# hdm0922/PathTracerDemo

Hardware: AMD Instinct MI355X
Metric: Msamples/sec at 1920x1080, 1 spp ReSTIR DI; per-pixel L2 vs WebGPU ref (higher is better)
Workload: dtype f32; 1 GPU; c3_interior_32 reuse 1920x1080, 1 spp/frame (configs[2]); frame=1920x1080, band_rows_per_gpu=1080, parallelism=row-bands x1

## Files before the change

### pathtracerdemo_amd/csrc/ptx_launch.h

```cpp
#pragma once

#include <hip/hip_runtime.h>

#include "ptx_device.h"

namespace ptx {

constexpr int kTile = 16;
constexpr int kBlock = 256;

int env_knob(const char *key, int dflt);
#ifdef PTX_AB_BUILD
inline int ab_knob(const char *key, int dflt) { return env_knob(key, dflt); }
#else
constexpr int ab_knob(const char *, int dflt) { return dflt; }
#endif

inline size_t stack_lds_bytes(uint32_t depth) { return (size_t)depth * kBlock * sizeof(uint32_t); }

hipError_t launch_gbuffer(const Scene &sc, uint4 *gbuf, uint32_t stack_depth, hipStream_t s);
hipError_t launch_init(const Scene &sc, const uint4 *gbuf, uint4 *reservoir, uint32_t stack_depth, hipStream_t s);
hipError_t launch_final(const Scene &sc, const uint4 *gbuf, const uint4 *reservoir, float4 *accum,
                        uint32_t stack_depth, hipStream_t s);
hipError_t launch_mcpt(const Scene &sc, float4 *accum, uint32_t stack_depth, hipStream_t s);
hipError_t launch_present(const float4 *tex, uint32_t W, uint32_t H, uint32_t cw, uint32_t ch, bool bgra,
                          uint32_t *out, hipStream_t s);

hipError_t launch_trace_rays(const Scene &sc, const float4 *rays, float4 *hits, uint32_t n, int eps_mode,
                             uint32_t stack_depth, hipStream_t s);

constexpr uint32_t kWaveStateSlots = 10u;
constexpr uint32_t kStateCs2 = 7u, kStateCs3 = 8u, kStateTsel = 9u;
constexpr uint32_t kWaveSegPixels = 768u;
constexpr int kWaveRoundsInit = 3, kWaveRoundsFinal = 3, kWaveRoundsMcpt = 4;
constexpr int kWaveMaxRounds = 5;
constexpr uint32_t kDynHeads = 8u, kDynStride = 32u;
constexpr uint32_t kDynRoundWords = kDynHeads * kDynStride;
constexpr uint32_t kDynCounters = 2u * 4u * kWaveMaxRounds * kDynRoundWords;
struct WaveBufs {
    float4 *state;
    uint32_t npix;
    uint32_t seg_px;
    uint32_t nseg;
    uint32_t seg_base;
    uint32_t seg_count;
    uint32_t cluster;
    uint32_t ray_stride;
    float4 *rays;
    float4 *res[3];
    uint32_t nres;
    uint32_t *act[2];
    uint32_t act_stride;
    uint32_t *cnt;
    uint32_t trace_waves;
    uint32_t trace_split;
// ... 75 lines not shown
```

### pathtracerdemo_amd/csrc/ptx_reuse.hip

```cpp
#include "ptx_wave_common.h"

namespace ptx {

constexpr uint32_t SALT_TEMPORAL = 0x54454D50u, SALT_SPATIAL = 0x53504154u;

enum : uint32_t { JS_HDR, JS_F, JS_CUR, JS_NRM, JS_PREV, JS_RRF, JS_COUNT };
constexpr uint32_t kJobFresh = 1u << 24;
constexpr uint32_t kResReuseLayout = 0x100u;
#ifndef PTX_JOB_FRESH
#define PTX_JOB_FRESH 1
#endif

struct Job {
    uint32_t i, length, phase, seed1, idx, matref;
    uint32_t k, lab;
    bool shift, rok;
    int32_t ref;
    int32_t dom;
    f3 f;
    float prod;
    Surface cur;
    f3 prev;
    float beta, rr_p;
    f3 rr_f;
// ... 62 lines not shown
    } else if (s.phase != 1u) {
        const float4 cu = st[JS_CUR * n + jid], nr = st[JS_NRM * n + jid];
        const float4 pv = st[JS_PREV * n + jid], rf = st[JS_RRF * n + jid];
        matref = asu(cu.w);
        cur.pos = mk(cu.x, cu.y, cu.z);
        cur.nrm = mk(nr.x, nr.y, nr.z);
        cur.mat = material_at(sc, matref);
        beta = nr.w;
        prev = mk(pv.x, pv.y, pv.z); rr_p = pv.w;
        rr_f = mk(rf.x, rf.y, rf.z);
    }
    s.seed1 = seed1; s.matref = matref; s.dom = dom;
    s.f = f; s.rr_f = rr_f; s.prev = prev;
    s.beta = beta; s.rr_p = rr_p;
    s.cur = cur;
}

__device__ __forceinline__ bool rr_step(Job &s, const Surface &X, f3 L, f3 fv, float pdf) {
    s.rr_f = s.rr_f * (fv * fabsf(dot(X.nrm, L)));
    s.rr_p *= pdf;
    const float ps = luminance(s.rr_f) / s.rr_p;
    const bool ok = ps > 0.0f;
    s.rr_p *= ps;
    if (ps > 1.0f) s.beta /= ps;
    return ok;
}

__device__ __forceinline__ void job_init(Job &s, f3 x0, const Surface &X1, uint32_t matref, int32_t ref,
                                         uint32_t length, uint32_t seed1, int32_t dom, uint32_t k, bool shift) {
    s.i = 1u; s.length = length; s.phase = 0u; s.seed1 = seed1; s.idx = 0u; s.ref = ref; s.dom = dom;
    s.k = min(k, 7u); s.lab = 0u; s.shift = shift; s.rok = false;
    s.f = mk(1.0f, 1.0f, 1.0f); s.prod = 1.0f;
    s.prev = x0;
    s.cur = X1;
    s.matref = matref;
    s.beta = 1.0f; s.rr_p = 1.0f; s.rr_f = mk(1.0f, 1.0f, 1.0f);
}
__device__ __forceinline__ bool job_begin(const Scene &sc, const ReuseArgs &A, Job &s, uint32_t x, uint32_t y,
                                          int32_t dom, int32_t ref) {
    const uint4 *rv = res_at(A.cur, ref);
    const uint4 r5 = rv[5];
    const uint32_t C = rv[7].y, length = r5.w;
    Surface X1;
    uint32_t matref;
    if (C == 0u || length < 2u || !surf_load(sc, A.surf, dom, X1, matref)) return false;
    job_init(s, x0_of(sc, x, y), X1, matref, ref, length, rv[0].y, dom, r5.x & 0xffu, false);
    return true;
// ... 217 lines not shown
__device__ __forceinline__ void write_reused(uint4 *out, const uint4 *src, float p_sel, float q_sel, SelF fs,
                                             float w_sum, uint32_t C) {
    uint4 a0 = src[0], a5 = src[5];
    const uint4 a1 = src[1], a2 = src[2], a3 = src[3], a4 = src[4];
    if (fs.known && !(a5.x & kResReuseLayout)) {
        const uint32_t k = a5.x & 0xffu;
        if (k >= 2u && k + 1u < a5.w) a0 = src[6];
        a5.x |= kResReuseLayout;
    }
    out[0] = a0; out[1] = a1; out[2] = a2; out[3] = a3; out[4] = a4; out[5] = a5;
    out[6] = make_uint4(asu(p_sel), asu(q_sel), fs.known ? asu(fs.f.x) : 0u, fs.known ? asu(fs.f.y) : 0u);
    out[7] = make_uint4(asu(p_sel > 0.0f ? w_sum / p_sel : 0.0f), C, fs.known ? asu(fs.f.z) : 0u, fs.known ? 1u : 0u);
}

constexpr uint32_t kNbrEscape = 0xFFFFFFFFu;
__device__ __forceinline__ uint4 nbr_pack(bool valid, uint4 r5, uint4 r6, uint4 r7) {
    uint32_t w = 0u;
    const uint32_t k = r5.x & 0xffu;
    if (valid)
        w = (r5.w > 0xfu || k > 0xfu || r7.y > 0x7ffffeu) ? kNbrEscape : (1u << 31) | (r5.w << 27) | (k << 23) | r7.y;
    return make_uint4(r6.x, r6.y, r7.x, w);
}

__device__ __forceinline__ bool temporal_from_init(const Scene &sc, const WaveBufs &w, const ReuseArgs &A, Job &s,
                                                   uint32_t pix, uint32_t jid) {
    const uint4 *rv = res_at(A.cur, s.ref);
    const bool hyb = job_hyb(s);
    while (s.i + 1u < s.length) {
        f3 V = normalize(s.prev - s.cur.pos);
        uint32_t seed = s.i == 1u ? rv[0].x : s.seed1, lobe;
        const f3 dir = sample_bsdf(seed, s.cur, V, lobe);
        float pdf;
        const f3 fv = bsdf_pdf(s.cur, V, dir, pdf);
        if (!hyb || s.i + 2u <= s.k) s.prod *= pdf;
        if (!rr_step(s, s.cur, dir, fv, pdf)) {
            A.jres[jid] = make_float4(0.0f, 0.0f, 0.0f, 0.0f);
            return false;
        }
        const float4 c = w.state[(s.i == 1u ? kStateCs2 : kStateCs3) * w.npix + pix];
        const Surface next = get_surface(sc, gdecode(make_uint4(asu(c.x), asu(c.y), asu(c.z), asu(c.w))));
        V = normalize(s.prev - s.cur.pos);
        const f3 L = normalize(next.pos - s.cur.pos);
        s.f = s.f * (bsdf(s.cur, L, V) * fabsf(dot(s.cur.nrm, L)));
        if (hyb && s.i + 1u == s.k) s.prod = s.prod * rc_geo(s.cur.pos, next);
        s.prev = s.cur.pos;
        s.cur = next;
        s.i += 1u;
    }
    const float T = w.state[kStateTsel * w.npix + pix].x;
    if (T < 0.0f) return true;
    const LightSample XL = load_xl(rv);
    const f3 V = normalize(s.prev - s.cur.pos);
    const f3 L = direction_to_light(s.cur, XL);
    s.f = s.f * (bsdf(s.cur, L, V) * fabsf(dot(s.cur.nrm, L)));
    float gl = 1.0f;
    if (XL.type == LIGHT_RECT) {
        const f3 r = XL.pos - s.cur.pos;
        const f3 Ld = normalize(r);
        gl = fabsf(dot(get_light(sc, (uint32_t)XL.id).dir, Ld)) / dot(r, r);
    }
    s.prod = hyb ? s.prod / s.beta : s.prod / (gl * s.beta);
    const f3 Le = l_emit<true>(XL, s.cur);
    s.f = s.f * (Le * T);
    const float qv = s.prod;
    const bool valid = qv > 0.0f && qv <= 3.402823466e38f;
    A.jres[jid] = valid ? make_float4(s.f.x, s.f.y, s.f.z, qv) : make_float4(0.0f, 0.0f, 0.0f, 0.0f);
    return false;
}

__global__ __launch_bounds__(WB) __attribute__((amdgpu_waves_per_eu(2, 8)))
void wtemporal_start(Scene sc, WaveBufs w, ReuseArgs A) {
    PTX_WAVE_TIMER(sc, KID_TEMP_START | (w.seg_base ? 0x80u : 0u));
    __shared__ uint32_t lds[3];
    const JobLists JL = job_lists(w, lds);
    const Seg g = seg_begin(w, 0u, lds);
    const uint32_t np = padded_pixels(sc);
    for (uint32_t k = 0; k < w.seg_px; k += WB) {
        const uint32_t q = seg_pixel(w, g.j, k);
        uint32_t x, y, pix = 0u;
        bool active = false;
        Job s;
        if (q < np && tile_xy(sc, q, x, y)) {
            pix = (y - sc.row_begin) * sc.width + x;
            active = job_begin(sc, A, s, x, y, (int32_t)pix, (int32_t)pix);
            if (active && A.use_init) active = temporal_from_init(sc, w, A, s, pix, pix);
        }
        const bool live = job_emit(sc, g, A, active, s, pix, active ? A.cur[8u * (size_t)pix].x : 0u);
        job_finish(g, JL, A, live, s, pix);
    }
    job_seg_end(w, g, JL);
}

__global__ __launch_bounds__(WB) void wtemporal_combine(Scene sc, WaveBufs w, ReuseArgs A) {
    PTX_WAVE_TIMER(sc, KID_TEMP_COMBINE | (w.seg_base ? 0x80u : 0u));
    const uint32_t j = w.seg_base + blockIdx.x, np = padded_pixels(sc);
    for (uint32_t k = 0; k < w.seg_px; k += WB) {
        const uint32_t q = seg_pixel(w, j, k);
        uint32_t x, y;
        if (q >= np || !tile_xy(sc, q, x, y)) continue;
        const uint32_t pix = (y - sc.row_begin) * sc.width + x;
        if (!gdecode(A.gbuf[pix]).valid) {
            A.nbr_out[pix] = make_uint4(0u, 0u, 0u, 0u);
            continue;
        }
        uint4 *rv = A.cur + 8u * (size_t)pix;
        const uint4 *hv = A.hist + 8u * (size_t)pix;
        uint32_t seed = reuse_seed(sc, x, y, SALT_TEMPORAL);
        const uint4 r5 = rv[5], r7 = rv[7];
        const float4 er = (r7.y != 0u && r5.w >= 2u) ? job_result(A, w, A.jres[pix], pix) : make_float4(0.0f, 0.0f, 0.0f, 0.0f);
        const float2 ec = make_float2(er.w > 0.0f ? luminance(mk(er.x, er.y, er.z)) : 0.0f, er.w);
        const bool canon_ok = ec.y > 0.0f && ec.x > 0.0f;
// ... 38 lines not shown
    m.py = (uint32_t)fy;
    const int32_t ry = (int32_t)m.py - (int32_t)sc.row_begin;
    if (abs((int32_t)m.py - (int32_t)y) > (int32_t)A.radius || ry < A.prev_row_lo || ry >= A.prev_row_hi) {
        if (count && A.clip) atomicAdd(A.clip, 1ull);
        return m;
    }
    m.pp = ry * (int32_t)sc.width + (int32_t)m.px;
    const uint4 a = A.psurf[2 * (ptrdiff_t)m.pp];
    if (a.w == kNoSurface) return m;
    const uint4 b = A.psurf[2 * (ptrdiff_t)m.pp + 1];
    const f3 pp = mk(asf(a.x), asf(a.y), asf(a.z)), pn = mk(asf(b.x), asf(b.y), asf(b.z));
    if (!(dot(pn, X1.nrm) >= 0.9f)) return m;
    const f3 x0p = x0_prev(A, sc, m.px, m.py);
    const float dp = length(pp - x0p), dc = length(P - x0p);
    if (!(fabsf(dp - dc) <= 0.05f * dc)) return m;
    m.C = min(A.hist[8 * (ptrdiff_t)m.pp + 7].y, A.cap);
    m.ok = m.C != 0u;
    return m;
}

#ifndef MOTION_START_WAVES
#define MOTION_START_WAVES 3
#endif
__global__ __launch_bounds__(WB) __attribute__((amdgpu_waves_per_eu(MOTION_START_WAVES, 8)))
void wtmotion_start(Scene sc, WaveBufs w, ReuseArgs A) {
    PTX_WAVE_TIMER(sc, KID_TEMP_START | (w.seg_base ? 0x80u : 0u));
    __shared__ uint32_t lds[3];
    const JobLists JL = job_lists(w, lds);
    const Seg g = seg_begin(w, 0u, lds);
    const uint32_t np = padded_pixels(sc);
    for (uint32_t k = 0; k < w.seg_px; k += WB) {
        const uint32_t q = seg_pixel(w, g.j, k);
        uint32_t x = 0u, y = 0u, pix = 0u;
        bool valid = false;
        Surface X1{};
        uint32_t mref = 0u;
        if (q < np && tile_xy(sc, q, x, y)) {
            pix = (y - sc.row_begin) * sc.width + x;
            valid = surf_load(sc, A.surf, pix, X1, mref);
        }
        const uint4 *rv = A.cur + 8u * (size_t)pix;
        const uint4 r5c = valid ? rv[5] : make_uint4(0u, 0u, 0u, 0u);
        const uint32_t cC = valid ? rv[7].y : 0u, clen = r5c.w, ck = r5c.x & 0xffu;
        const bool canon = valid && cC != 0u && clen >= 2u;
        const MotionHist mh = valid ? motion_hist(sc, A, X1, y, true) : MotionHist{false, 0, 0u, 0u, 0u};
#pragma unroll 1
        for (uint32_t slot = 0; slot < kMotionJobs; ++slot) {
            const uint32_t jid = job_id(A, pix, slot);
            Job s;
            bool act = false;
            uint32_t s0 = 0u;
            if (slot == 0u) {
                act = canon && job_begin(sc, A, s, x, y, (int32_t)pix, (int32_t)pix);
                if (act && A.use_init) act = temporal_from_init(sc, w, A, s, pix, jid);
                if (act) s0 = rv[0].x;
            } else if (slot == 1u) {
                if (mh.ok) {
                    const uint4 *hv = A.hist + 8 * (ptrdiff_t)mh.pp;
                    const uint4 h0 = hv[0], h5 = hv[5], h6 = hv[6];
                    act = h5.w >= 2u && asf(h6.x) > 0.0f;
                    if (act) {
                        job_init(s, x0_of(sc, x, y), X1, mref, kHistRef + mh.pp, h5.w, h0.y, (int32_t)pix, h5.x & 0xffu,
                                 true);
                        s0 = h0.x;
                    }
                }
            } else if (mh.ok && canon) {
                Surface Xp;
                uint32_t pref;
                act = surf_load(sc, A.psurf, mh.pp, Xp, pref);
                if (act) {
                    job_init(s, x0_prev(A, sc, mh.px, mh.py), Xp, pref, (int32_t)pix, clen, rv[0].y, kDomPrev, ck, true);
                    s0 = rv[0].x;
                }
            }
            const bool live = job_emit(sc, g, A, act, s, jid, s0);
            job_finish(g, JL, A, live, s, jid);
        }
    }
    job_seg_end(w, g, JL);
}

__global__ __launch_bounds__(WB) void wtmotion_combine(Scene sc, WaveBufs w, ReuseArgs A) {
    PTX_WAVE_TIMER(sc, KID_TEMP_COMBINE | (w.seg_base ? 0x80u : 0u));
    const uint32_t j = w.seg_base + blockIdx.x, np = padded_pixels(sc);
    for (uint32_t k = 0; k < w.seg_px; k += WB) {
        const uint32_t q = seg_pixel(w, j, k);
        uint32_t x, y;
        if (q >= np || !tile_xy(sc, q, x, y)) continue;
        const uint32_t pix = (y - sc.row_begin) * sc.width + x;
        Surface X1;
        uint32_t mref;
        if (!surf_load(sc, A.surf, pix, X1, mref)) {
            A.nbr_out[pix] = make_uint4(0u, 0u, 0u, 0u);
            continue;
        }
        uint4 *rv = A.cur + 8u * (size_t)pix;
        uint32_t seed = reuse_seed(sc, x, y, SALT_TEMPORAL);
        const uint4 r5 = rv[5], r7 = rv[7];
        const float4 er = (r7.y != 0u && r5.w >= 2u) ? job_at(A, w, pix, 0u) : make_float4(0.0f, 0.0f, 0.0f, 0.0f);
        const float ecp = er.w > 0.0f ? luminance(mk(er.x, er.y, er.z)) : 0.0f, ecq = er.w;
        const bool canon_ok = ecq > 0.0f && ecp > 0.0f;
        const float cc = 1.0f, pc = ecp, qc = ecq, Wc = asf(r7.x);
        const MotionHist mh = motion_hist(sc, A, X1, y);
// ... 90 lines not shown
    return hipGetLastError();
}

__global__ __launch_bounds__(WB) void wsurface(Scene sc, WaveBufs w, const uint4 *gbuf) {
    const uint32_t j = w.seg_base + blockIdx.x, np = padded_pixels(sc);
    for (uint32_t k = 0; k < w.seg_px; k += WB) {
        const uint32_t q = seg_pixel(w, j, k);
        uint32_t x, y;
        if (q >= np || !tile_xy(sc, q, x, y)) continue;
        const uint32_t pix = (y - sc.row_begin) * sc.width + x;
        surf_from_gbuf(sc, w.surf, (ptrdiff_t)pix, gbuf[pix]);
    }
}
hipError_t wave_surface(const Scene &sc, const WaveBufs &w, const uint4 *gbuf, hipStream_t s) {
    if (!w.surf || !w.seg_count) return hipSuccess;
    hipLaunchKernelGGL(wsurface, dim3(w.seg_count), dim3(WB), 0, s, sc, w, gbuf);
    return hipGetLastError();
}

constexpr uint32_t kMaxPrefetch = 3u;
#ifndef SPATIAL_START_WAVES
#define SPATIAL_START_WAVES 3
#endif
constexpr uint32_t kBinCap = 128u;
__device__ __forceinline__ uint32_t bin_push(uint4 *bin, uint32_t cnt, bool p, uint4 d) {
    const unsigned long long m = __ballot(p);
    const uint32_t rank = __builtin_amdgcn_mbcnt_hi((uint32_t)(m >> 32), __builtin_amdgcn_mbcnt_lo((uint32_t)m, 0u));
    if (p) bin[cnt + rank] = d;
    return cnt + (uint32_t)__popcll(m);
}
template <int KIND>
__device__ __forceinline__ void spatial_drain(const Scene &sc, const Seg &g, const JobLists &JL, const ReuseArgs &A,
                                              const uint4 *bin, uint32_t first, uint32_t n) {
    const uint32_t lane = threadIdx.x & 63u;
    const bool act = lane < n;
    uint32_t jid = 0u, s0 = 0u;
    Job s;
    if (act) {
        const uint4 d = bin[first + lane];
        const int32_t dom = (int32_t)d.x, ref = (int32_t)d.y;
        const uint32_t slot = d.w >> 16;
        jid = job_id(A, (slot & 1u) ? d.y : d.x, slot);
        Surface X1{};
        uint32_t mref = 0u;
        (void)surf_load(sc, A.surf, dom, X1, mref);
        const uint4 b = res_at(A.cur, ref)[0];
        job_init(s, x0_of(sc, d.z & 0xffffu, d.z >> 16), X1, mref, ref, d.w & 0xffu, b.y, dom, (d.w >> 8) & 0xffu, true);
        s0 = b.x;
    }
    const bool live = job_emit<KIND>(sc, g, A, act, s, jid, s0);
    job_finish(g, JL, A, live, s, jid);
}
__global__ __launch_bounds__(WB) __attribute__((amdgpu_waves_per_eu(SPATIAL_START_WAVES, 8)))
// ... 310 lines not shown
    for (uint32_t k = 0; k < w.seg_px; k += WB) {
        const uint32_t q = seg_pixel(w, j, k);
        uint32_t x, y;
        if (q >= np || !tile_xy(sc, q, x, y)) continue;
        const uint32_t pix = (y - sc.row_begin) * sc.width + x;
        if (!gdecode(A.gbuf[pix]).valid) {
            uint4 *out = A.hist + 8u * (size_t)pix;
            for (int t = 0; t < 8; ++t) out[t] = make_uint4(0u, 0u, 0u, 0u);
            continue;
        }
        if (A.neighbors == 3u) combine_pixel<3>(sc, A, w, x, y, pix);
        else combine_pixel<0>(sc, A, w, x, y, pix);
    }
}

int reuse_rounds(int pass_temporal, const ReuseArgs &A) {
    return pass_temporal && A.use_init && !A.motion ? 1 : kWaveRoundsReuse;
}

hipError_t wave_reuse_round(const Scene &sc, const WaveBufs &w, int pass_temporal, int round, const ReuseArgs &A,
                            hipStream_t s) {
    const dim3 grid(w.seg_count), blk(WB);
    if (round == 0) {
        if (pass_temporal && A.motion) hipLaunchKernelGGL(wtmotion_start, grid, blk, 0, s, sc, w, A);
        else if (pass_temporal) hipLaunchKernelGGL(wtemporal_start, grid, blk, 0, s, sc, w, A);
        else hipLaunchKernelGGL(wspatial_start, grid, blk, 0, s, sc, w, A);
    } else if (round <= reuse_rounds(pass_temporal, A)) {
        hipLaunchKernelGGL(wjob_step, grid, blk, 0, s, sc, w, (uint32_t)round, A);
    } else {
        if (pass_temporal && A.motion) hipLaunchKernelGGL(wtmotion_combine, grid, blk, 0, s, sc, w, A);
        else if (pass_temporal) hipLaunchKernelGGL(wtemporal_combine, grid, blk, 0, s, sc, w, A);
        else if (A.neighbors == 3u && !ab_knob("COMBINE_SCALAR", 0))
            hipLaunchKernelGGL(wspatial_combine_shfl, dim3(w.seg_count), blk, 0, s, sc, w, A);
        else hipLaunchKernelGGL(wspatial_combine, grid, blk, 0, s, sc, w, A);
    }
    return hipGetLastError();
}

}
```

### pathtracerdemo_amd/csrc/ptx_wave.hip

```cpp
#include "ptx_wave_common.h"

#include <algorithm>
#include <cstdlib>

namespace ptx {

#ifndef TRACE_OCC_WAVES
#define TRACE_OCC_WAVES 5
#endif
#ifndef TRACE_COOP
#define TRACE_COOP true
#endif
#ifndef PTX_NODE_UNI
#define PTX_NODE_UNI 1
#endif
#ifndef PTX_FLAT_INST
#define PTX_FLAT_INST 1
#endif
constexpr uint32_t kFlatMinInstances = 1u;
#ifndef PTX_LDS_TRANS
#define PTX_LDS_TRANS 1
#endif
template <bool COUNT, bool PROF, bool OCC, bool LDS_TABLES, bool FLAT>
__device__ __forceinline__ void trace_lanes(const Scene &sc, const SubRoot *subs, const Inst *insts, PassEps eps,
// ... 346 lines not shown
template <bool ROOTQ>
__global__ __launch_bounds__(WB) void wgbuffer(Scene sc, WaveBufs w, uint4 *gbuf) {
    PTX_WAVE_TIMER(sc, KID_GBUF);
    extern __shared__ __attribute__((aligned(16))) uint32_t wstack[];
    uint32_t *stack = wstack + tables_lds_bytes(sc) / 4u + threadIdx.x;
    const LdsTables T = stage_tables(sc, wstack);
    const uint32_t L = blockIdx.x * 4u + threadIdx.x / 64u, run = w.cluster * w.seg_count;
    const uint32_t t = set_tile(w, (L / run) * w.cluster * w.nseg + w.cluster * w.seg_base + L % run);
    const uint32_t q = t * 64u + (threadIdx.x & 63u);
    uint32_t x, y;
    if (q >= padded_pixels(sc) || !tile_xy(sc, q, x, y)) return;
    const float *vpinv = reinterpret_cast<const float *>(sc.U + U_VPINV);
    const float u = ((float)x + 0.5f) / (float)sc.U[U_W];
    const float v = ((float)y + 0.5f) / (float)sc.U[U_H];
    const f3 st = xform_point(vpinv, mk(2.0f * u - 1.0f, 2.0f * v - 1.0f, 0.0f));
    const f3 en = xform_point(vpinv, mk(2.0f * u - 1.0f, 2.0f * v - 1.0f, 0.0f + 1.0f));
    const Hit h = trace_core_tab<false, false, ROOTQ>(sc, T.subs, T.insts, Ray{st, normalize(en - st)},
                                                      PassEps{1e-8f, 1e-6f}, stack, WB);
    Compact c = h.s;
    c.valid = h.valid ? 1u : 0u;
    gbuf[(y - sc.row_begin) * sc.width + x] = gencode(c);
}

enum : uint32_t { IS_HDR, IS_FP, IS_RES, IS_X, IS_XL, IS_L, IS_BSEED, IS_CS2, IS_CS3, IS_TSEL, IS_COUNT };
static_assert(IS_CS2 == kStateCs2 && IS_CS3 == kStateCs3 && IS_TSEL == kStateTsel && IS_COUNT <= kWaveStateSlots,
              "PT_1 state slots read by the temporal pass (ptx_reuse.hip)");
enum : uint32_t { F_SEL = 1u, F_BSDF = 2u, F_FAR12 = 4u, F_FAR23 = 8u, F_R1 = 16u, F_R2 = 32u };

struct WInit {
    uint32_t seed, i, flags, C, vis_idx, bsdf_idx;
    f3 f; float p;
    float w_sum, p_hat_sel, pdf_env;
    f3 xpos; float xrough;
    f3 xlpos; uint32_t nee_seed;
    f3 L;
    uint32_t bseed1, bseed2;
};
__device__ __forceinline__ uint32_t lobe_of(uint32_t flags, uint32_t k) { return (flags >> (8u + 2u * (k - 1u))) & 3u; }

__device__ __forceinline__ void wcompress(const Scene &sc, const WInit &s, const float4 *state, uint32_t npix,
                                          uint32_t pix, bool is_env, const LightSample &XL, uint4 *out,
                                          bool rcnext) {
    const uint32_t i = s.i, length = i + 1u;
    const uint32_t L1 = (i > 1u || is_env) ? lobe_of(s.flags, 1u) : 0u;
    const uint32_t L2 = (i > 2u || (is_env && i == 2u)) ? lobe_of(s.flags, 2u) : 0u;
    const uint32_t s2 = (i >= 2u || is_env) ? s.bseed1 : s.nee_seed;
    const uint32_t s3 = (i >= 3u || (i == 2u && is_env)) ? s.bseed2 : (i == 2u ? s.nee_seed : 0u);
    const uint32_t s4 = (i == 3u) ? s.nee_seed : 0u;
    uint32_t k = 0u;
    if (length > 2u) {
        bool ok = (L1 == LOBE_LAMBERT || (s.flags & F_R1)) && (L2 == LOBE_LAMBERT || (s.flags & F_R2));
        if ((s.flags & F_FAR12) && ok) k = 2u;
    }
    if (k == 0u && length > 3u) {
        bool ok = (L2 == LOBE_LAMBERT || (s.flags & F_R2));
        if ((s.flags & F_FAR23) && ok) k = 3u;
    }
    if (k == 0u) {
        bool rough = s.xrough >= RECONNECTION_ROUGHNESS;
// ... 9 lines not shown
        lk = L2; lk1 = L1;
        const float4 c = state[IS_CS2 * npix + pix];
        rc = make_uint4(asu(c.x), asu(c.y), asu(c.z), asu(c.w));
    } else if (k == 3u) {
        lk1 = L2;
        const float4 c = state[IS_CS3 * npix + pix];
        rc = make_uint4(asu(c.x), asu(c.y), asu(c.z), asu(c.w));
    }
    out[0] = make_uint4(s2, s3, s4, 0u);
    out[1] = make_uint4(asu(XL.dir.x), asu(XL.dir.y), asu(XL.dir.z), XL.type);
    out[2] = make_uint4(asu(XL.pos.x), asu(XL.pos.y), asu(XL.pos.z), (uint32_t)XL.id);
    out[3] = make_uint4(asu(XL.Le.x), asu(XL.Le.y), asu(XL.Le.z), asu(XL.pdf));
    out[4] = rc;
    out[5] = make_uint4(k, lk1, lk, length);
    uint4 nx = make_uint4(0u, 0u, 0u, 0u);
    if (rcnext && k == 2u && length == 4u) {
        const float4 c = state[IS_CS3 * npix + pix];
        nx = make_uint4(asu(c.x), asu(c.y), asu(c.z), asu(c.w));
    }
    out[6] = nx;
}

__device__ __forceinline__ void winit_vertex(const Scene &sc, const Seg &g, bool emit, WInit &s, const Surface &X,
                                             f3 prev) {
    float4 *rays = g.rays, *res = g.res_out;
    const uint32_t vbase = g.rbase + wave_alloc(g.l_ray, emit ? 1u : 0u);
    bool bsdf_ray = false;
    if (emit) {
        const f3 V = normalize(prev - X.pos);
        s.nee_seed = s.seed;
        const LightSample XL = sample_nee(sc, s.seed, X, V);
        const f3 Ln = direction_to_light(X, XL);
        f3 contrib = s.f * l_emit<false>(XL, X);
        contrib = contrib * bsdf(X, V, Ln);
        contrib = contrib * fabsf(dot(X.nrm, Ln));
        const float denom = s.p * XL.pdf;
        const float u_update = rnd(s.seed);
        s.xlpos = XL.pos;
        s.xpos = X.pos;
        s.xrough = X.mat.rough;
        s.vis_idx = vbase;
        const float dist = length(XL.pos - X.pos);
        put_ray(rays, vbase, X.pos, (XL.pos - X.pos) / dist, dist, Q_VIS);
        res[2u * vbase] = make_float4(0.0f, contrib.x, contrib.y, contrib.z);
        res[2u * vbase + 1u] = make_float4(denom, u_update, XL.pdf, asf((uint32_t)XL.id));
        if (s.i < 3u) {
            if (s.i == 1u) s.bseed1 = s.seed;
            else s.bseed2 = s.seed;
            uint32_t lobe;
            const f3 Lb = sample_bsdf(s.seed, X, V, lobe);
            s.flags |= lobe << (8u + 2u * (s.i - 1u));
            float pdfv;
            const f3 bv = bsdf_pdf(X, V, Lb, pdfv);
            s.f = s.f * (bv * fabsf(dot(X.nrm, Lb)));
            s.p *= pdfv;
            const float ps = luminance(s.f) / s.p;
            if (rnd(s.seed) < ps) {
                s.p *= ps;
                s.pdf_env = pdfv;
                s.L = Lb;
                bsdf_ray = true;
            }
        }
        s.flags = bsdf_ray ? (s.flags | F_BSDF) : (s.flags & ~F_BSDF);
    }
    const uint32_t bbase = g.rbase + wave_alloc(g.l_ray, bsdf_ray ? 1u : 0u);
    if (bsdf_ray) {
        s.bsdf_idx = bbase;
        put_ray(rays, bbase, s.xpos, s.L, -1.0f, Q_CLOSEST);
    }
}

__device__ __forceinline__ void winit_store(float4 *state, uint32_t npix, uint32_t pix, const WInit &s) {
    state[IS_HDR * npix + pix] = make_float4(asf(s.seed), asf(s.i | (s.flags << 8)), asf(s.C), asf(s.vis_idx));
    state[IS_FP * npix + pix] = make_float4(s.f.x, s.f.y, s.f.z, s.p);
    state[IS_RES * npix + pix] = make_float4(s.w_sum, s.p_hat_sel, s.pdf_env, asf(s.bsdf_idx));
    state[IS_X * npix + pix] = make_float4(s.xpos.x, s.xpos.y, s.xpos.z, s.xrough);
    state[IS_XL * npix + pix] = make_float4(s.xlpos.x, s.xlpos.y, s.xlpos.z, asf(s.nee_seed));
    state[IS_L * npix + pix] = make_float4(s.L.x, s.L.y, s.L.z, 0.0f);
    state[IS_BSEED * npix + pix] = make_float4(asf(s.bseed1), asf(s.bseed2), 0.0f, 0.0f);
}
__device__ __forceinline__ void winit_load(const float4 *state, uint32_t npix, uint32_t pix, WInit &s) {
    const float4 h = state[IS_HDR * npix + pix], fp = state[IS_FP * npix + pix], r = state[IS_RES * npix + pix];
    const float4 x = state[IS_X * npix + pix], xl = state[IS_XL * npix + pix], l = state[IS_L * npix + pix];
    const float4 b = state[IS_BSEED * npix + pix];
    s.seed = asu(h.x); s.i = asu(h.y) & 0xffu; s.flags = asu(h.y) >> 8; s.C = asu(h.z); s.vis_idx = asu(h.w);
    s.f = mk(fp.x, fp.y, fp.z); s.p = fp.w;
    s.w_sum = r.x; s.p_hat_sel = r.y; s.pdf_env = r.z; s.bsdf_idx = asu(r.w);
    s.xpos = mk(x.x, x.y, x.z); s.xrough = x.w;
    s.xlpos = mk(xl.x, xl.y, xl.z); s.nee_seed = asu(xl.w);
    s.L = mk(l.x, l.y, l.z);
    s.bseed1 = asu(b.x); s.bseed2 = asu(b.y);
}
__device__ __forceinline__ void winit_finish(const WInit &s, uint4 *reservoir, uint32_t pix) {
    uint4 *out = reservoir + 8u * (size_t)pix;
    if (!(s.flags & F_SEL))
        for (int q = 0; q < 7; ++q) out[q] = make_uint4(0u, 0u, 0u, 0u);
    out[7] = make_uint4(asu(s.w_sum / s.p_hat_sel), s.C, 0u, 0u);
}

__global__ __launch_bounds__(WB) __attribute__((amdgpu_waves_per_eu(LOGIC_WAVES, 8))) void winit_start(Scene sc, WaveBufs w, const uint4 *gbuf, uint4 *reservoir) {
    PTX_WAVE_TIMER(sc, KID_INIT_START | (w.seg_base ? 0x80u : 0u));
    __shared__ uint32_t lds[3];
    const JobLists JL = job_lists(w, lds);
    const Seg g = seg_begin(w, 0u, lds);
    float4 *state = w.state;
    const uint32_t npix = w.npix, np = padded_pixels(sc);
    for (uint32_t k = 0; k < w.seg_px; k += WB) {
        const uint32_t q = seg_pixel(w, g.j, k);
        uint32_t x, y, pix = 0u;
        bool active = false;
        WInit s;
        Surface X;
        f3 prev;
        if (q < np && tile_xy(sc, q, x, y)) {
            pix = (y - sc.row_begin) * sc.width + x;
            const Compact x1 = gdecode(gbuf[pix]);
            if (!x1.valid) {
                uint4 *out = reservoir + 8u * (size_t)pix;
                for (int q8 = 0; q8 < 8; ++q8) out[q8] = make_uint4(0u, 0u, 0u, 0u);
                if (w.surf) surf_store_none(w.surf, pix);
            } else {
                active = true;
                s.seed = pcg(x * 1973u + y * 9277u + sc.U[U_FRAME] * 26699u);
                s.i = 1u; s.flags = 0u; s.C = 0u;
                s.f = mk(1.0f, 1.0f, 1.0f); s.p = 1.0f;
                s.w_sum = 0.0f; s.p_hat_sel = 0.0f; s.pdf_env = 0.0f;
                s.L = mk(0.0f, 0.0f, 0.0f); s.bseed1 = 0u; s.bseed2 = 0u; s.bsdf_idx = 0u;
                prev = x0_of(sc, x, y);
                X = get_surface(sc, x1);
                if (w.surf) surf_store(w.surf, pix, X, mat_index(sc, x1.inst, x1.mat));
                if (X.mat.rough >= RECONNECTION_ROUGHNESS) s.flags |= F_R1;
            }
        }
        winit_vertex(sc, g, active, s, X, prev);
        if (active) winit_store(state, npix, pix, s);
        job_keep(g, JL, active, active && !(s.flags & F_BSDF), pix);
    }
    job_seg_end(w, g, JL);
}

__global__ __launch_bounds__(WB) __attribute__((amdgpu_waves_per_eu(LOGIC_WAVES, 8))) void winit_step(Scene sc, WaveBufs w, uint32_t round, uint4 *reservoir) {
    PTX_WAVE_TIMER(sc, KID_INIT_STEP | (w.seg_base ? 0x80u : 0u));
    __shared__ uint32_t lds[3];
    const JobLists JL = job_lists(w, lds);
    const Seg g = seg_begin(w, round, lds);
    float4 *state = w.state;
    const float4 *res_in = g.res_in;
    const uint32_t npix = w.npix;
    uint32_t nh;
    const uint32_t n = split_count(g, nh);
    for (uint32_t base = 0; base < n; base += WB) {
        const uint32_t q = base + threadIdx.x;
        bool emit = false;
        uint32_t pix = 0u;
        WInit s;
        Surface X;
        f3 prev;
        if (q < n) {
// ... 44 lines not shown
                        env.Le = mk(ENV_C, ENV_C, ENV_C);
                        env.pdf = s.pdf_env;
                        wcompress(sc, s, state, npix, pix, true, env, reservoir + 8u * (size_t)pix, w.surf != nullptr);
                    }
                    winit_finish(s, reservoir, pix);
                } else {
                    X = surface_at(sc, h.s, h.pos);
                    prev = s.xpos;
                    s.i += 1u;
                    if (s.i == 2u) {
                        if (length3(prev - X.pos) >= RECONNECTION_DISTANCE) s.flags |= F_FAR12;
                        if (X.mat.rough >= RECONNECTION_ROUGHNESS) s.flags |= F_R2;
                        const uint4 e = gencode(h.s);
                        state[IS_CS2 * npix + pix] = make_float4(asf(e.x), asf(e.y), asf(e.z), asf(e.w));
                    } else {
                        if (length3(prev - X.pos) >= RECONNECTION_DISTANCE) s.flags |= F_FAR23;
                        const uint4 e = gencode(h.s);
                        state[IS_CS3 * npix + pix] = make_float4(asf(e.x), asf(e.y), asf(e.z), asf(e.w));
                    }
                    emit = true;
                }
            }
        }
        winit_vertex(sc, g, emit, s, X, prev);
        if (emit) winit_store(state, npix, pix, s);
        job_keep(g, JL, emit, emit && !(s.flags & F_BSDF), pix);
    }
    job_seg_end(w, g, JL);
}

enum : uint32_t { FS_HDR, FS_F, FS_CUR, FS_NRM, FS_PREV, FS_COUNT };

struct WFinal {
    uint32_t i, length, phase, seed1, idx;
    f3 f; float ucw;
    Surface cur;
    f3 prev;
};
__device__ __forceinline__ void wfinal_emit(const Scene &sc, const Seg &g, bool emit, WFinal &s, const uint4 *resv) {
    float4 *rays = g.rays, *res = g.res_out;
    const uint32_t idx = g.rbase + wave_alloc(g.l_ray, emit ? 1u : 0u);
    if (!emit) return;
    const f3 V = normalize(s.prev - s.cur.pos);
    s.idx = idx;
    if (s.i + 1u < s.length) {
        uint32_t seed = s.i == 1u ? resv[0].x : s.seed1;
        uint32_t lobe;
        const f3 dir = sample_bsdf(seed, s.cur, V, lobe);
// ... 536 lines not shown
```

### pathtracerdemo_amd/csrc/ptx_wave_common.h

```cpp
#pragma once
#include "ptx_launch.h"
#include "ptx_shading.h"

namespace ptx {

constexpr uint32_t WB = kBlock;
#ifndef LOGIC_WAVES
#define LOGIC_WAVES 4
#endif
enum : uint32_t { Q_CLOSEST = 0u, Q_VIS = 1u, Q_OCC = 2u };

__device__ __forceinline__ uint32_t wave_scan(uint32_t v, uint32_t &total) { return wave_excl_sum(v, total); }
__device__ __forceinline__ uint32_t wave_alloc(uint32_t *lds_ctr, uint32_t n) {
    uint32_t total;
    const uint32_t excl = wave_scan(n, total);
    uint32_t base = 0u;
    if (__lane_id() == 0u && total) base = atomicAdd(lds_ctr, total);
    base = (uint32_t)__builtin_amdgcn_readfirstlane((int)base);
    return base + excl;
}

struct Seg {
    uint32_t j, round;
    uint32_t pj;
// ... 123 lines not shown
    surf[2 * i] = make_uint4(asu(X.pos.x), asu(X.pos.y), asu(X.pos.z), matref);
    surf[2 * i + 1] = make_uint4(asu(X.nrm.x), asu(X.nrm.y), asu(X.nrm.z), 0u);
}
__device__ __forceinline__ void surf_store_none(uint4 *surf, ptrdiff_t i) {
    surf[2 * i] = make_uint4(0u, 0u, 0u, kNoSurface);
}
__device__ __forceinline__ bool surf_load(const Scene &sc, const uint4 *surf, ptrdiff_t i, Surface &X,
                                          uint32_t &matref) {
    const uint4 a = surf[2 * i];
    if (a.w == kNoSurface) return false;
    const uint4 b = surf[2 * i + 1];
    X.pos = mk(asf(a.x), asf(a.y), asf(a.z));
    X.nrm = mk(asf(b.x), asf(b.y), asf(b.z));
    X.mat = material_at(sc, a.w);
    matref = a.w;
    return true;
}
__device__ __forceinline__ void surf_from_gbuf(const Scene &sc, uint4 *surf, ptrdiff_t i, uint4 g) {
    const Compact x1 = gdecode(g);
    if (!x1.valid) surf_store_none(surf, i);
    else surf_store(surf, i, get_surface(sc, x1), mat_index(sc, x1.inst, x1.mat));
}

__device__ __forceinline__ LightSample load_xl(const uint4 *res) {
    const uint4 r1 = res[1], r2 = res[2], r3 = res[3];
    LightSample XL;
    XL.dir = mk(asf(r1.x), asf(r1.y), asf(r1.z));
    XL.type = r1.w;
    XL.pos = mk(asf(r2.x), asf(r2.y), asf(r2.z));
    XL.id = (int32_t)r2.w;
    XL.Le = mk(asf(r3.x), asf(r3.y), asf(r3.z));
    XL.pdf = asf(r3.w);
    return XL;
}
}
```

Baseline: 568.9 Msamples/s.

## Hand over init-pass BSDF pdf and RR beta to temporal reuse instead of replaying

```diff
diff --git a/pathtracerdemo_amd/csrc/ptx_launch.h b/pathtracerdemo_amd/csrc/ptx_launch.h
--- a/pathtracerdemo_amd/csrc/ptx_launch.h
+++ b/pathtracerdemo_amd/csrc/ptx_launch.h
@@ -29,8 +29,8 @@
 hipError_t launch_trace_rays(const Scene &sc, const float4 *rays, float4 *hits, uint32_t n, int eps_mode,
                              uint32_t stack_depth, hipStream_t s);
 
-constexpr uint32_t kWaveStateSlots = 10u;
-constexpr uint32_t kStateCs2 = 7u, kStateCs3 = 8u, kStateTsel = 9u;
+constexpr uint32_t kWaveStateSlots = 11u;
+constexpr uint32_t kStateCs2 = 7u, kStateCs3 = 8u, kStateTsel = 9u, kStateHand = 10u;
 constexpr uint32_t kWaveSegPixels = 768u;
 constexpr int kWaveRoundsInit = 3, kWaveRoundsFinal = 3, kWaveRoundsMcpt = 4;
 constexpr int kWaveMaxRounds = 5;
diff --git a/pathtracerdemo_amd/csrc/ptx_reuse.hip b/pathtracerdemo_amd/csrc/ptx_reuse.hip
--- a/pathtracerdemo_amd/csrc/ptx_reuse.hip
+++ b/pathtracerdemo_amd/csrc/ptx_reuse.hip
@@ -108,7 +108,7 @@
     const float ps = luminance(s.rr_f) / s.rr_p;
     const bool ok = ps > 0.0f;
     s.rr_p *= ps;
-    if (ps > 1.0f) s.beta /= ps;
+    s.beta = rr_beta(s.beta, ps);
     return ok;
 }
 
@@ -372,24 +372,45 @@
     return make_uint4(r6.x, r6.y, r7.x, w);
 }
 
+constexpr uint32_t kBinCap = 128u;
+template <typename D>
+__device__ __forceinline__ uint32_t bin_push(D *bin, uint32_t cnt, bool p, D d) {
+    const unsigned long long m = __ballot(p);
+    const uint32_t rank = __builtin_amdgcn_mbcnt_hi((uint32_t)(m >> 32), __builtin_amdgcn_mbcnt_lo((uint32_t)m, 0u));
+    if (p) bin[cnt + rank] = d;
+    return cnt + (uint32_t)__popcll(m);
+}
+
+enum : int { TI_REPLAY = 0, TI_HANDED = 1, TI_ENV = 2, TI_BY_T = 3 };
+template <int MODE>
 __device__ __forceinline__ bool temporal_from_init(const Scene &sc, const WaveBufs &w, const ReuseArgs &A, Job &s,
-                                                   uint32_t pix, uint32_t jid) {
+                                                   uint32_t pix, uint32_t jid, float T) {
     const uint4 *rv = res_at(A.cur, s.ref);
     const bool hyb = job_hyb(s);
+    const bool replay = MODE == TI_REPLAY || MODE == TI_ENV || (MODE == TI_BY_T && T < 0.0f);
     while (s.i + 1u < s.length) {
-        f3 V = normalize(s.prev - s.cur.pos);
-        uint32_t seed = s.i == 1u ? rv[0].x : s.seed1, lobe;
-        const f3 dir = sample_bsdf(seed, s.cur, V, lobe);
-        float pdf;
-        const f3 fv = bsdf_pdf(s.cur, V, dir, pdf);
-        if (!hyb || s.i + 2u <= s.k) s.prod *= pdf;
-        if (!rr_step(s, s.cur, dir, fv, pdf)) {
-            A.jres[jid] = make_float4(0.0f, 0.0f, 0.0f, 0.0f);
-            return false;
+        const f3 V = normalize(s.prev - s.cur.pos);
+        if (replay) {
+            uint32_t seed = s.i == 1u ? rv[0].x : s.seed1, lobe;
+            const f3 dir = sample_bsdf(seed, s.cur, V, lobe);
+            float pdf;
+            const f3 fv = bsdf_pdf(s.cur, V, dir, pdf);
+            if (!hyb || s.i + 2u <= s.k) s.prod *= pdf;
+            if (!rr_step(s, s.cur, dir, fv, pdf)) {
+                A.jres[jid] = make_float4(0.0f, 0.0f, 0.0f, 0.0f);
+                return false;
+            }
+        } else {
+            const float2 hand = hand_plane(w.state, w.npix, min(s.i, 2u))[pix];
+            if (!hyb || s.i + 2u <= s.k) s.prod *= hand.x;
+            s.beta = hand_beta(hand.y);
+            if (!hand_ok(hand.y)) {
+                A.jres[jid] = make_float4(0.0f, 0.0f, 0.0f, 0.0f);
+                return false;
+            }
         }
         const float4 c = w.state[(s.i == 1u ? kStateCs2 : kStateCs3) * w.npix + pix];
         const Surface next = get_surface(sc, gdecode(make_uint4(asu(c.x), asu(c.y), asu(c.z), asu(c.w))));
-        V = normalize(s.prev - s.cur.pos);
         const f3 L = normalize(next.pos - s.cur.pos);
         s.f = s.f * (bsdf(s.cur, L, V) * fabsf(dot(s.cur.nrm, L)));
         if (hyb && s.i + 1u == s.k) s.prod = s.prod * rc_geo(s.cur.pos, next);
@@ -397,8 +418,7 @@
         s.cur = next;
         s.i += 1u;
     }
-    const float T = w.state[kStateTsel * w.npix + pix].x;
-    if (T < 0.0f) return true;
+    if (MODE == TI_ENV || T < 0.0f) return true;
     const LightSample XL = load_xl(rv);
     const f3 V = normalize(s.prev - s.cur.pos);
     const f3 L = direction_to_light(s.cur, XL);
@@ -418,10 +438,9 @@
     return false;
 }
 
-__global__ __launch_bounds__(WB) __attribute__((amdgpu_waves_per_eu(2, 8)))
-void wtemporal_start(Scene sc, WaveBufs w, ReuseArgs A) {
-    PTX_WAVE_TIMER(sc, KID_TEMP_START | (w.seg_base ? 0x80u : 0u));
-    __shared__ uint32_t lds[3];
+template <bool REPLAY>
+__device__ __forceinline__ void temporal_start_segment(const Scene &sc, const WaveBufs &w, const ReuseArgs &A,
+                                                       uint32_t *lds) {
     const JobLists JL = job_lists(w, lds);
     const Seg g = seg_begin(w, 0u, lds);
     const uint32_t np = padded_pixels(sc);
@@ -433,10 +452,97 @@
         if (q < np && tile_xy(sc, q, x, y)) {
             pix = (y - sc.row_begin) * sc.width + x;
             active = job_begin(sc, A, s, x, y, (int32_t)pix, (int32_t)pix);
-            if (active && A.use_init) active = temporal_from_init(sc, w, A, s, pix, pix);
-        }
-        const bool live = job_emit(sc, g, A, active, s, pix, active ? A.cur[8u * (size_t)pix].x : 0u);
+            if (REPLAY && active)
+                active = temporal_from_init<TI_REPLAY>(sc, w, A, s, pix, pix,
+                                                       w.state[kStateTsel * w.npix + pix].x);
+        }
+        const bool live = job_emit<REPLAY ? JK_L : JK_ANY>(sc, g, A, active, s, pix,
+                                                           !REPLAY && active ? A.cur[8u * (size_t)pix].x : 0u);
         job_finish(g, JL, A, live, s, pix);
+    }
+    job_seg_end(w, g, JL);
+}
+__global__ __launch_bounds__(WB) __attribute__((amdgpu_waves_per_eu(JOB_STEP_WAVES, 8)))
+void wtemporal_start_cold(Scene sc, WaveBufs w, ReuseArgs A) {
+    PTX_WAVE_TIMER(sc, KID_TEMP_START | (w.seg_base ? 0x80u : 0u));
+    __shared__ uint32_t lds[3];
+    temporal_start_segment<false>(sc, w, A, lds);
+}
+#ifdef PTX_AB_BUILD
+__global__ __launch_bounds__(WB) __attribute__((amdgpu_waves_per_eu(2, 8)))
+void wtemporal_start_replay(Scene sc, WaveBufs w, ReuseArgs A) {
+    PTX_WAVE_TIMER(sc, KID_TEMP_START | (w.seg_base ? 0x80u : 0u));
+    __shared__ uint32_t lds[3];
+    temporal_start_segment<true>(sc, w, A, lds);
+}
+#endif
+
+__global__ __launch_bounds__(WB) __attribute__((amdgpu_waves_per_eu(4, 8)))
+void wtemporal_start(Scene sc, WaveBufs w, ReuseArgs A) {
+    PTX_WAVE_TIMER(sc, KID_TEMP_START | (w.seg_base ? 0x80u : 0u));
+    const uint32_t j = w.seg_base + blockIdx.x, np = padded_pixels(sc);
+    for (uint32_t k = 0; k < w.seg_px; k += WB) {
+        const uint32_t q = seg_pixel(w, j, k);
+        uint32_t x, y;
+        if (q >= np || !tile_xy(sc, q, x, y)) continue;
+        const uint32_t pix = (y - sc.row_begin) * sc.width + x;
+        const float T = w.state[kStateTsel * w.npix + pix].x;
+        Job s;
+        if (!(T < 0.0f) && job_begin(sc, A, s, x, y, (int32_t)pix, (int32_t)pix))
+            (void)temporal_from_init<TI_HANDED>(sc, w, A, s, pix, pix, T);
+    }
+}
+constexpr uint32_t kEnvBlock = 64u, kEnvAhead = 4u;
+__global__ __launch_bounds__(kEnvBlock) __attribute__((amdgpu_waves_per_eu(3, 8)))
+void wtemporal_env(Scene sc, WaveBufs w, ReuseArgs A) {
+    PTX_WAVE_TIMER(sc, KID_TEMP_START | (w.seg_base ? 0x80u : 0u));
+    __shared__ uint32_t lds[3];
+    __shared__ uint2 bin[kBinCap];
+    const JobLists JL = job_lists(w, lds);
+    const Seg g = seg_begin(w, 0u, lds);
+    const uint32_t np = padded_pixels(sc), lane = threadIdx.x;
+    uint32_t cnt = 0u;
+    for (uint32_t k = 0; k < w.seg_px + kEnvAhead * 64u; k += kEnvAhead * 64u) {
+        const bool flush = k >= w.seg_px;
+        uint2 dv[kEnvAhead];
+        float Tv[kEnvAhead];
+#pragma unroll
+        for (uint32_t u = 0; u < kEnvAhead; ++u) {
+            const uint32_t q = k + 64u * u < w.seg_px ? seg_pixel(w, g.j, k + 64u * u) : np;
+            uint32_t x, y;
+            dv[u] = make_uint2(0u, 0u);
+            Tv[u] = 0.0f;
+            if (q < np && tile_xy(sc, q, x, y)) {
+                dv[u] = make_uint2((y - sc.row_begin) * sc.width + x, x | (y << 16));
+                Tv[u] = w.state[kStateTsel * w.npix + dv[u].x].x;
+            }
+        }
+#pragma unroll 1
+        for (uint32_t u = 0; u < kEnvAhead; ++u) {
+            uint2 d = dv[0];
+            float T = Tv[0];
+#pragma unroll
+            for (uint32_t v = 1; v < kEnvAhead; ++v)
+                if (v == u) { d = dv[v]; T = Tv[v]; }
+            cnt = bin_push(bin, cnt, T < 0.0f, d);
+            __builtin_amdgcn_fence(__ATOMIC_ACQ_REL, "wavefront");
+            if (cnt >= (flush ? 1u : 64u)) {
+                const uint32_t n = min(cnt, 64u);
+                cnt -= n;
+                uint32_t pix = 0u;
+                bool active = false;
+                Job s;
+                if (lane < n) {
+                    const uint2 e = bin[cnt + lane];
+                    pix = e.x;
+                    active = job_begin(sc, A, s, e.y & 0xffffu, e.y >> 16, (int32_t)pix, (int32_t)pix) &&
+                             temporal_from_init<TI_ENV>(sc, w, A, s, pix, pix, -1.0f);
+                }
+                const bool live = job_emit<JK_L>(sc, g, A, active, s, pix, 0u);
+                job_finish(g, JL, A, live, s, pix);
+            }
+            __builtin_amdgcn_fence(__ATOMIC_ACQ_REL, "wavefront");
+        }
     }
     job_seg_end(w, g, JL);
 }
@@ -521,10 +627,9 @@
 #ifndef MOTION_START_WAVES
 #define MOTION_START_WAVES 3
 #endif
-__global__ __launch_bounds__(WB) __attribute__((amdgpu_waves_per_eu(MOTION_START_WAVES, 8)))
-void wtmotion_start(Scene sc, WaveBufs w, ReuseArgs A) {
-    PTX_WAVE_TIMER(sc, KID_TEMP_START | (w.seg_base ? 0x80u : 0u));
-    __shared__ uint32_t lds[3];
+template <bool HAND>
+__device__ __forceinline__ void tmotion_start_segment(const Scene &sc, const WaveBufs &w, const ReuseArgs &A,
+                                                      uint32_t *lds) {
     const JobLists JL = job_lists(w, lds);
     const Seg g = seg_begin(w, 0u, lds);
     const uint32_t np = padded_pixels(sc);
@@ -551,7 +656,9 @@
             uint32_t s0 = 0u;
             if (slot == 0u) {
                 act = canon && job_begin(sc, A, s, x, y, (int32_t)pix, (int32_t)pix);
-                if (act && A.use_init) act = temporal_from_init(sc, w, A, s, pix, jid);
+                if (act && A.use_init)
+                    act = temporal_from_init<HAND ? TI_BY_T : TI_REPLAY>(sc, w, A, s, pix, jid,
+                                                                        w.state[kStateTsel * w.npix + pix].x);
                 if (act) s0 = rv[0].x;
             } else if (slot == 1u) {
                 if (mh.ok) {
@@ -579,6 +686,20 @@
     }
     job_seg_end(w, g, JL);
 }
+__global__ __launch_bounds__(WB) __attribute__((amdgpu_waves_per_eu(MOTION_START_WAVES, 8)))
+void wtmotion_start(Scene sc, WaveBufs w, ReuseArgs A) {
+    PTX_WAVE_TIMER(sc, KID_TEMP_START | (w.seg_base ? 0x80u : 0u));
+    __shared__ uint32_t lds[3];
+    tmotion_start_segment<true>(sc, w, A, lds);
+}
+#ifdef PTX_AB_BUILD
+__global__ __launch_bounds__(WB) __attribute__((amdgpu_waves_per_eu(MOTION_START_WAVES, 8)))
+void wtmotion_start_replay(Scene sc, WaveBufs w, ReuseArgs A) {
+    PTX_WAVE_TIMER(sc, KID_TEMP_START | (w.seg_base ? 0x80u : 0u));
+    __shared__ uint32_t lds[3];
+    tmotion_start_segment<false>(sc, w, A, lds);
+}
+#endif
 
 __global__ __launch_bounds__(WB) void wtmotion_combine(Scene sc, WaveBufs w, ReuseArgs A) {
     PTX_WAVE_TIMER(sc, KID_TEMP_COMBINE | (w.seg_base ? 0x80u : 0u));
@@ -715,13 +836,6 @@
 #ifndef SPATIAL_START_WAVES
 #define SPATIAL_START_WAVES 3
 #endif
-constexpr uint32_t kBinCap = 128u;
-__device__ __forceinline__ uint32_t bin_push(uint4 *bin, uint32_t cnt, bool p, uint4 d) {
-    const unsigned long long m = __ballot(p);
-    const uint32_t rank = __builtin_amdgcn_mbcnt_hi((uint32_t)(m >> 32), __builtin_amdgcn_mbcnt_lo((uint32_t)m, 0u));
-    if (p) bin[cnt + rank] = d;
-    return cnt + (uint32_t)__popcll(m);
-}
 template <int KIND>
 __device__ __forceinline__ void spatial_drain(const Scene &sc, const Seg &g, const JobLists &JL, const ReuseArgs &A,
                                               const uint4 *bin, uint32_t first, uint32_t n) {
@@ -1078,9 +1192,24 @@
                             hipStream_t s) {
     const dim3 grid(w.seg_count), blk(WB);
     if (round == 0) {
-        if (pass_temporal && A.motion) hipLaunchKernelGGL(wtmotion_start, grid, blk, 0, s, sc, w, A);
-        else if (pass_temporal) hipLaunchKernelGGL(wtemporal_start, grid, blk, 0, s, sc, w, A);
-        else hipLaunchKernelGGL(wspatial_start, grid, blk, 0, s, sc, w, A);
+#ifdef PTX_AB_BUILD
+        static const bool replay = ab_knob("TEMPORAL_HANDOVER", 1) == 0;
+        if (pass_temporal && replay && (A.motion || A.use_init)) {
+            if (A.motion) hipLaunchKernelGGL(wtmotion_start_replay, grid, blk, 0, s, sc, w, A);
+            else hipLaunchKernelGGL(wtemporal_start_replay, grid, blk, 0, s, sc, w, A);
+            return hipGetLastError();
+        }
+#endif
+        if (pass_temporal && A.motion) {
+            hipLaunchKernelGGL(wtmotion_start, grid, blk, 0, s, sc, w, A);
+        } else if (pass_temporal && A.use_init) {
+            hipLaunchKernelGGL(wtemporal_start, grid, blk, 0, s, sc, w, A);
+            hipLaunchKernelGGL(wtemporal_env, grid, dim3(kEnvBlock), 0, s, sc, w, A);
+        } else if (pass_temporal) {
+            hipLaunchKernelGGL(wtemporal_start_cold, grid, blk, 0, s, sc, w, A);
+        } else {
+            hipLaunchKernelGGL(wspatial_start, grid, blk, 0, s, sc, w, A);
+        }
     } else if (round <= reuse_rounds(pass_temporal, A)) {
         hipLaunchKernelGGL(wjob_step, grid, blk, 0, s, sc, w, (uint32_t)round, A);
     } else {
diff --git a/pathtracerdemo_amd/csrc/ptx_wave.hip b/pathtracerdemo_amd/csrc/ptx_wave.hip
--- a/pathtracerdemo_amd/csrc/ptx_wave.hip
+++ b/pathtracerdemo_amd/csrc/ptx_wave.hip
@@ -392,8 +392,9 @@
     gbuf[(y - sc.row_begin) * sc.width + x] = gencode(c);
 }
 
-enum : uint32_t { IS_HDR, IS_FP, IS_RES, IS_X, IS_XL, IS_L, IS_BSEED, IS_CS2, IS_CS3, IS_TSEL, IS_COUNT };
-static_assert(IS_CS2 == kStateCs2 && IS_CS3 == kStateCs3 && IS_TSEL == kStateTsel && IS_COUNT <= kWaveStateSlots,
+enum : uint32_t { IS_HDR, IS_FP, IS_RES, IS_X, IS_XL, IS_L, IS_BSEED, IS_CS2, IS_CS3, IS_TSEL, IS_HAND, IS_COUNT };
+static_assert(IS_CS2 == kStateCs2 && IS_CS3 == kStateCs3 && IS_TSEL == kStateTsel && IS_HAND == kStateHand &&
+                  IS_COUNT <= kWaveStateSlots,
               "PT_1 state slots read by the temporal pass (ptx_reuse.hip)");
 enum : uint32_t { F_SEL = 1u, F_BSDF = 2u, F_FAR12 = 4u, F_FAR23 = 8u, F_R1 = 16u, F_R2 = 32u };
 
@@ -405,6 +406,7 @@
     f3 xlpos; uint32_t nee_seed;
     f3 L;
     uint32_t bseed1, bseed2;
+    float hbeta;
 };
 __device__ __forceinline__ uint32_t lobe_of(uint32_t flags, uint32_t k) { return (flags >> (8u + 2u * (k - 1u))) & 3u; }
 
@@ -460,7 +462,7 @@
 }
 
 __device__ __forceinline__ void winit_vertex(const Scene &sc, const Seg &g, bool emit, WInit &s, const Surface &X,
-                                             f3 prev) {
+                                             f3 prev, float &hpdf) {
     float4 *rays = g.rays, *res = g.res_out;
     const uint32_t vbase = g.rbase + wave_alloc(g.l_ray, emit ? 1u : 0u);
     bool bsdf_ray = false;
@@ -493,6 +495,8 @@
             s.f = s.f * (bv * fabsf(dot(X.nrm, Lb)));
             s.p *= pdfv;
             const float ps = luminance(s.f) / s.p;
+            hpdf = pdfv;
+            s.hbeta = hand_pack(hand_beta(s.hbeta), ps);
             if (rnd(s.seed) < ps) {
                 s.p *= ps;
                 s.pdf_env = pdfv;
@@ -515,7 +519,7 @@
     state[IS_RES * npix + pix] = make_float4(s.w_sum, s.p_hat_sel, s.pdf_env, asf(s.bsdf_idx));
     state[IS_X * npix + pix] = make_float4(s.xpos.x, s.xpos.y, s.xpos.z, s.xrough);
     state[IS_XL * npix + pix] = make_float4(s.xlpos.x, s.xlpos.y, s.xlpos.z, asf(s.nee_seed));
-    state[IS_L * npix + pix] = make_float4(s.L.x, s.L.y, s.L.z, 0.0f);
+    state[IS_L * npix + pix] = make_float4(s.L.x, s.L.y, s.L.z, s.hbeta);
     state[IS_BSEED * npix + pix] = make_float4(asf(s.bseed1), asf(s.bseed2), 0.0f, 0.0f);
 }
 __device__ __forceinline__ void winit_load(const float4 *state, uint32_t npix, uint32_t pix, WInit &s) {
@@ -527,7 +531,7 @@
     s.w_sum = r.x; s.p_hat_sel = r.y; s.pdf_env = r.z; s.bsdf_idx = asu(r.w);
     s.xpos = mk(x.x, x.y, x.z); s.xrough = x.w;
     s.xlpos = mk(xl.x, xl.y, xl.z); s.nee_seed = asu(xl.w);
-    s.L = mk(l.x, l.y, l.z);
+    s.L = mk(l.x, l.y, l.z); s.hbeta = l.w;
     s.bseed1 = asu(b.x); s.bseed2 = asu(b.y);
 }
 __device__ __forceinline__ void winit_finish(const WInit &s, uint4 *reservoir, uint32_t pix) {
@@ -564,15 +568,19 @@
                 s.i = 1u; s.flags = 0u; s.C = 0u;
                 s.f = mk(1.0f, 1.0f, 1.0f); s.p = 1.0f;
                 s.w_sum = 0.0f; s.p_hat_sel = 0.0f; s.pdf_env = 0.0f;
-                s.L = mk(0.0f, 0.0f, 0.0f); s.bseed1 = 0u; s.bseed2 = 0u; s.bsdf_idx = 0u;
+                s.L = mk(0.0f, 0.0f, 0.0f); s.bseed1 = 0u; s.bseed2 = 0u; s.bsdf_idx = 0u; s.hbeta = 1.0f;
                 prev = x0_of(sc, x, y);
                 X = get_surface(sc, x1);
                 if (w.surf) surf_store(w.surf, pix, X, mat_index(sc, x1.inst, x1.mat));
                 if (X.mat.rough >= RECONNECTION_ROUGHNESS) s.flags |= F_R1;
             }
         }
-        winit_vertex(sc, g, active, s, X, prev);
-        if (active) winit_store(state, npix, pix, s);
+        float hpdf = 0.0f;
+        winit_vertex(sc, g, active, s, X, prev, hpdf);
+        if (active) {
+            winit_store(state, npix, pix, s);
+            if (w.surf) hand_plane(state, npix, 1u)[pix] = make_float2(hpdf, s.hbeta);
+        }
         job_keep(g, JL, active, active && !(s.flags & F_BSDF), pix);
     }
     job_seg_end(w, g, JL);
@@ -663,8 +671,12 @@
                 }
             }
         }
-        winit_vertex(sc, g, emit, s, X, prev);
-        if (emit) winit_store(state, npix, pix, s);
+        float hpdf = 0.0f;
+        winit_vertex(sc, g, emit, s, X, prev, hpdf);
+        if (emit) {
+            winit_store(state, npix, pix, s);
+            if (w.surf && s.i == 2u) hand_plane(state, npix, 2u)[pix] = make_float2(hpdf, s.hbeta);
+        }
         job_keep(g, JL, emit, emit && !(s.flags & F_BSDF), pix);
     }
     job_seg_end(w, g, JL);
diff --git a/pathtracerdemo_amd/csrc/ptx_wave_common.h b/pathtracerdemo_amd/csrc/ptx_wave_common.h
--- a/pathtracerdemo_amd/csrc/ptx_wave_common.h
+++ b/pathtracerdemo_amd/csrc/ptx_wave_common.h
@@ -169,6 +169,19 @@
     else surf_store(surf, i, get_surface(sc, x1), mat_index(sc, x1.inst, x1.mat));
 }
 
+__device__ __forceinline__ float2 *hand_plane(float4 *state, uint32_t npix, uint32_t vertex) {
+    return reinterpret_cast<float2 *>(state + (size_t)kStateHand * npix) + (size_t)(vertex - 1u) * npix;
+}
+__device__ __forceinline__ float rr_beta(float beta, float ps) {
+    if (ps > 1.0f) beta /= ps;
+    return beta;
+}
+__device__ __forceinline__ float hand_pack(float beta_before, float ps) {
+    return asf(asu(rr_beta(beta_before, ps)) | (ps > 0.0f ? 0u : 0x80000000u));
+}
+__device__ __forceinline__ bool hand_ok(float b) { return (asu(b) >> 31) == 0u; }
+__device__ __forceinline__ float hand_beta(float b) { return asf(asu(b) & 0x7fffffffu); }
+
 __device__ __forceinline__ LightSample load_xl(const uint4 *res) {
     const uint4 r1 = res[1], r2 = res[2], r3 = res[3];
     LightSample XL;
```

Result: no change. 566.4 Msamples/s (-0.4%).
